# rafaelsoStanford/State_Policy_DiffusionModel

Measured on AMD Instinct MI355X. Metric: denoise-steps/sec (B=4096, horizon=32), higher is better.
Workload: dtype f32 (split-fp16 MFMA operands, fp32 accumulate)

## Files before the change

### state_policy_diffusionmodel_amd/csrc/conv_gemm.hip

```cpp
#include <algorithm>
#include <cstdlib>

#include "device_utils.h"

namespace spdm {

typedef float f32x16 __attribute__((ext_vector_type(16)));
typedef float f32x4 __attribute__((ext_vector_type(4)));
typedef float f32x2 __attribute__((ext_vector_type(2)));
typedef unsigned u32x2 __attribute__((ext_vector_type(2)));
typedef _Float16 f16x8 __attribute__((ext_vector_type(8)));
typedef _Float16 f16x4 __attribute__((ext_vector_type(4)));

constexpr float SPLIT_ACT_SCALE = 16.0f;
constexpr float SPLIT_DESCALE = 1.0f / 2048.0f;

typedef _Float16 f16x2 __attribute__((ext_vector_type(2)));
__device__ __forceinline__ f32x2 split_pair(float a, float b) {
    unsigned h, l;
    split_pair_f16(a * SPLIT_ACT_SCALE, b * SPLIT_ACT_SCALE, h, l);
    return f32x2{__builtin_bit_cast(float, h), __builtin_bit_cast(float, l)};
}

constexpr int CK = 32;
// ... 443 lines not shown
#undef SPDM_TRANSFORM_A_X
#undef SPDM_WRITE_A_X
#undef SPDM_DMA_W
#undef SPDM_WOFF
#undef SPDM_LOAD_A
#undef SPDM_LOAD_W
#undef SPDM_STORE_W
#undef SPDM_TRANSFORM_A
#undef SPDM_WRITE_A

    if (PREC == PREC_SPLIT) {
#pragma unroll
        for (int mt = 0; mt < MT; ++mt)
#pragma unroll
            for (int nt = 0; nt < NT; ++nt)
#pragma unroll
                for (int r = 0; r < 16; ++r) acc[mt][nt][r] *= SPLIT_DESCALE;
    }

    SPDM_STAMP()
    float* srow = smem;
    constexpr int SROW_FLOATS = M_T * WN * 2;
    float* otile = smem + SROW_FLOATS;
    const bool unit4 = !W2 && (HW & 3) == 0;
#pragma unroll
    for (int mt = 0; mt < MT; ++mt)
#pragma unroll
        for (int nt = 0; nt < NT; ++nt) {
            const int col_l = wn * NT * 32 + nt * 32 + li;
#pragma unroll
            for (int r = 0; r < 16; ++r) {
                const int row_l = SPDM_ROW(mt, (r & 3) + 8 * (r >> 2) + 4 * kh);
                otile[row_l * N_T + col_l] = acc[mt][nt][r];
            }
        }

    const int epi = (ksp > 1) ? EPI_PLAIN : a.epi;
    float* const dstp = (ksp > 1) ? a.partial + (size_t)ks * M * N : a.dst;
    const int dst_ld = (ksp > 1) ? N : a.dst_ld;
    if (epi == EPI_STATS) {
#pragma unroll
        for (int mt = 0; mt < MT; ++mt)
#pragma unroll
            for (int g = 0; g < 4; ++g) {
                const int r0 = wm * MT * 32 + mt * 32 + 8 * g + 4 * kh;
                if (unit4) {
                    float s1 = 0.f, s2 = 0.f;
#pragma unroll
                    for (int nt = 0; nt < NT; ++nt)
#pragma unroll
                        for (int j = 0; j < 4; ++j) {
                            const float v = acc[mt][nt][4 * g + j];
                            s1 += v;
                            s2 += v * v;
                        }
                    s1 = half_sum(s1);
                    s2 = half_sum(s2);
                    if (li == 0) {
                        srow[((r0 >> 2) * WN + wn) * 2] = s1;
                        srow[((r0 >> 2) * WN + wn) * 2 + 1] = s2;
                    }
                } else {
#pragma unroll
                    for (int j = 0; j < 4; ++j) {
                        float s1 = 0.f, s2 = 0.f;
#pragma unroll
                        for (int nt = 0; nt < NT; ++nt) {
                            const float v = acc[mt][nt][4 * g + j];
                            s1 += v;
                            s2 += v * v;
                        }
                        s1 = half_sum(s1);
                        s2 = half_sum(s2);
                        if (li == 0) {
                            const int rr = SPDM_ROW(mt, 8 * g + 4 * kh + j);
                            srow[(rr * WN + wn) * 2] = s1;
                            srow[(rr * WN + wn) * 2 + 1] = s2;
                        }
                    }
                }
            }
    }
    SPDM_STAMP()
    __syncthreads();
    SPDM_STAMP()

    if (epi == EPI_STATS) {
        const int t_lo = m0, t_hi = min(m0 + M_T, M);
        if (t_hi > t_lo) {
            const int b_first = t_lo / HW, b_last = (t_hi - 1) / HW;
            const int ush = unit4 ? 2 : 0;
            for (int t = tid; t <= b_last - b_first; t += NTHR) {
                const int b = b_first + t;
                const int r_lo = max(b * HW, t_lo) - m0, r_hi = min((b + 1) * HW, t_hi) - m0;
                double s1 = 0.0, s2 = 0.0;
                for (int u = r_lo >> ush; u < ((r_hi + (unit4 ? 3 : 0)) >> ush); ++u)
                    for (int w2 = 0; w2 < WN; ++w2) {
                        s1 += (double)srow[(u * WN + w2) * 2];
                        s2 += (double)srow[(u * WN + w2) * 2 + 1];
                    }
                const int slot = (mtile - (b * HW) / M_T) * n_ntiles + ntile;
                double* o = a.epi_stats + ((size_t)b * epi_slots + slot) * 2;
                o[0] = s1;
                o[1] = s2;
            }
        }
    }

    {
        constexpr int TPR = N_T / 4, RPP = NTHR / TPR;
        const int c4o = tid % TPR, r0 = tid / TPR;
        const bool has_bias = (epi == EPI_BIAS || epi == EPI_BIAS_GELU || epi == EPI_BIAS_RESID);
        f32x4 bias4 = {0.f, 0.f, 0.f, 0.f};
        if (has_bias) bias4 = *reinterpret_cast<const f32x4*>(a.bias + n0 + c4o * 4);
#pragma unroll 4
        for (int p = 0; p < M_T / RPP; ++p) {
            const int row_l = p * RPP + r0;
            const int row = m0 + row_l;
            if (row < M && !(dbg & DBG_NO_STORE)) {
                f32x4 v = *reinterpret_cast<const f32x4*>(otile + row_l * N_T + c4o * 4);
                v += bias4;
                if (epi == EPI_BIAS_GELU) {
                    v.x = gelu_erf(v.x); v.y = gelu_erf(v.y); v.z = gelu_erf(v.z); v.w = gelu_erf(v.w);
                }
                if (epi == EPI_BIAS_RESID)
                    v += *reinterpret_cast<const f32x4*>(a.resid + (size_t)row * a.resid_ld + n0 + c4o * 4);
                *reinterpret_cast<f32x4*>(dstp + (size_t)row * dst_ld + n0 + c4o * 4) = v;
                if (a.row_stats != nullptr) {
                    float s1 = (v.x + v.y) + (v.z + v.w);
                    float s2 = (v.x * v.x + v.y * v.y) + (v.z * v.z + v.w * v.w);
#pragma unroll
                    for (int o2 = TPR >> 1; o2 > 0; o2 >>= 1) {
                        s1 += __shfl_xor(s1, o2, 64);
                        s2 += __shfl_xor(s2, o2, 64);
                    }
                    if (c4o == 0) {
                        double* rs = a.row_stats + ((size_t)row * n_ntiles + ntile) * 2;
                        rs[0] = (double)s1;
                        rs[1] = (double)s2;
                    }
                }
            }
        }
    }
    SPDM_STAMP()
#ifdef SPDM_DIAG
    if (stamping) a.stamps[(tid >> 8) * 128 + 127] = (unsigned long long)nstamp;
#endif
#undef SPDM_STAMP
#undef SPDM_ROW
}

int spdm_tune(int idx, int dflt) {
    constexpr int NT = 24;
    static int val[NT];
    static bool have[NT], init = false;
    if (!init) {
        for (int i = 0; i < NT; ++i) {
            char name[20];
            snprintf(name, sizeof(name), "SPDM_TUNE%d", i);
            const char* e = getenv(name);
            have[i] = e != nullptr;
            val[i] = e ? atoi(e) : 0;
        }
        init = true;
    }
    return (idx >= 0 && idx < NT && have[idx]) ? val[idx] : dflt;
}

GemmGeom gemm_geometry(int M, int N, int K, int HW, int W, int taps, int split, unsigned sw, bool stats_epi) {
    GemmGeom g;
    g.skinny = 0;
    g.reg = 0;
    if (stats_epi && conv_reg_geometry(M, N, K, HW, W, taps, split, sw)) {
        g.reg = 1;
        g.m_tile = 64; g.n_tile = 64; g.n_tiles = 1; g.ksplit = 1;
        g.st_m_tile = 64; g.st_n_tiles = 1;
        g.slots = stats_slots(HW, 64, 1);
        return g;
    }
    if (stats_epi && taps != 1 && conv_skinny_geometry(M, N, K, HW, W, taps, split, sw, &g.m_tile, &g.n_tile)) {
        g.skinny = 1;
        g.ksplit = 1;
        g.n_tiles = N / g.n_tile;
        g.st_m_tile = g.m_tile;
        g.st_n_tiles = g.n_tiles;
        g.slots = stats_slots(HW, g.st_m_tile, g.st_n_tiles);
        return g;
    }
    if (stats_epi && split && taps != 1 && spdm_tune(5, 0) > 0) {
        g.m_tile = spdm_tune(5, 0);
        g.n_tile = spdm_tune(6, 64);
        g.ksplit = std::max(1, spdm_tune(7, 1));
        if (N % g.n_tile != 0 || (g.m_tile != 128 && g.m_tile != 256)) { g.n_tile = 64; g.m_tile = 128; }
        g.n_tiles = N / g.n_tile;
        if (g.ksplit > K / CK) g.ksplit = K / CK;
        while (g.ksplit > 1 && (size_t)g.ksplit * M * N * sizeof(float) > SPLITK_WORKSPACE_BYTES) --g.ksplit;
        if (g.ksplit > 1) { g.st_m_tile = combine_rows(HW, N); g.st_n_tiles = 1; }
        else { g.st_m_tile = g.m_tile; g.st_n_tiles = g.n_tiles; }
        g.slots = stats_slots(HW, g.st_m_tile, g.st_n_tiles);
        return g;
    }
    const int nt128 = (N % 128 == 0) ? N / 128 : 0;
    const int nt_pref = nt128 ? nt128 : N / 64;
    bool big = split && taps != 1 && M >= 256;
    if (big && (long long)((M + 255) / 256) * nt_pref < spdm_tune(4, nt128 ? 257 : 192)) big = false;
    if (big && taps == 3 && HW % 4 == 0 && (long long)((M + 255) / 256) * nt_pref < 512 && !(sw & SW_T3_BIG)) big = false;
    g.m_tile = big ? 256 : 128;
    g.n_tile = nt128 ? 128 : 64;
    if (!big && nt128 && (long long)((M + 127) / 128) * nt128 < 192) g.n_tile = 64;
    if (big && g.n_tile == 64 && taps == 9 && (long long)((M + 511) / 512) * (N / 64) >= 192 &&
        !(sw & SW_NO_T512) && ((HW & 3) != 0 || (sw & SW_T512)))
        g.m_tile = 512;
    g.n_tiles = N / g.n_tile;
    g.ksplit = 1;
    const bool may_split = stats_epi && split && taps != 1 && K % CK == 0 && !(sw & SW_NO_SPLITK);
    if (may_split && !big && split && taps == 9 && W == 2 && (HW & 7) == 0 && M >= 256 && K % 64 == 0 && K >= 256 && spdm_tune(2, 1) != 0) {
        const long long t256 = (long long)((M + 255) / 256) * nt_pref;
        const int target = spdm_tune(0, 256);
        int S = (int)std::min<long long>(K / 64, (target + t256 - 1) / t256);
        while (S > 1 && (size_t)S * M * N * sizeof(float) > SPLITK_WORKSPACE_BYTES) --S;
        if (t256 * S >= target * 3 / 4 && S <= spdm_tune(3, 8)) {
            g.m_tile = 256; g.n_tile = nt128 ? 128 : 64; g.n_tiles = N / g.n_tile; g.ksplit = S;
            if (S > 1) { g.st_m_tile = combine_rows(HW, N); g.st_n_tiles = 1; }
            else { g.st_m_tile = g.m_tile; g.st_n_tiles = g.n_tiles; }
            g.slots = stats_slots(HW, g.st_m_tile, g.st_n_tiles);
            return g;
        }
    }
    if (may_split && !big) {
        const int nchunks = K / CK;
        const int target = spdm_tune(0, 256);
        const bool wide128 = nt128 && (HW & 3) == 0 && K % 64 == 0 && !(sw & (SW_NO_WIDE | SW_NO_WIDE128)) && spdm_tune(1, 0) != 0;
        const long long mt = (M + 127) / 128;
        if (wide128 && mt * nt128 < target) g.n_tile = 128, g.n_tiles = nt128;
        const long long tiles = mt * g.n_tiles;
        if (tiles < target) {
            const bool pairs = g.n_tile == 128 && (HW & 3) == 0 && K % 64 == 0 && !(sw & (SW_NO_WIDE | SW_NO_WIDE128));
            const int unit = pairs ? 2 : 1;
            int S = (int)std::min<long long>(nchunks / unit, (target + tiles - 1) / tiles);
            while (S > 1 && (size_t)S * M * N * sizeof(float) > SPLITK_WORKSPACE_BYTES) --S;
            if (S > 1) g.ksplit = S;
        }
    }
    if (g.ksplit > 1) {
        g.st_m_tile = combine_rows(HW, N);
        g.st_n_tiles = 1;
    } else {
        g.st_m_tile = g.m_tile;
        g.st_n_tiles = g.n_tiles;
    }
    g.slots = stats_slots(HW, g.st_m_tile, g.st_n_tiles);
    return g;
}

GemmGeom gemm_geometry(const GemmArgs& a) {
    return gemm_geometry(a.geom_M > 0 ? a.geom_M : a.M, a.N, a.K, a.HW, a.W, a.taps, a.split, a.sw, a.epi == EPI_STATS && a.partial != nullptr);
}

bool gemm_takes_fused_source(const GemmArgs& a) {
    if (!(a.pro == PRO_POOL || a.pro == PRO_UPCAT) || !a.split || a.wgt_frag == nullptr || (a.sw & SW_NO_FUSED_SRC) || a.epi != EPI_STATS) return false;
    if (a.pro == PRO_UPCAT && (a.up_C <= 0 || a.up_C >= a.K || a.up_C % CK != 0 || (a.H & 1) || (a.W & 1))) return false;
    const GemmGeom g = gemm_geometry(a);
    if (g.skinny != 0) return true;
    if (a.pro != PRO_UPCAT || g.reg || g.ksplit > 1) return false;
    GemmArgs b = a;
    b.ksplit = 1;
    return conv_wide_takes_upcat(b, g);
}

bool gemm_takes_two_sources(const GemmArgs& a0) {
    if (a0.skip == nullptr || !a0.split || a0.wgt_frag == nullptr || (a0.sw & SW_NO_FUSED_SRC) || a0.epi != EPI_STATS) return false;
    GemmArgs a = a0;
    const GemmGeom g = gemm_geometry(a);
    if (g.skinny || g.reg || g.m_tile == 512) return false;
    a.ksplit = g.ksplit;
    return conv_wide_supported(a, g);
}

static bool uses_w2(const GemmArgs& a, const GemmGeom& g) {
    return a.split && g.m_tile == 256 && a.taps == 9 && a.W == 2 && a.HW % 2 == 0 && !(a.sw & SW_NO_W2);
}
static bool uses_wp4(const GemmArgs& a0, const GemmGeom& g) {
    if (!(a0.split && a0.taps == 9 && a0.W == 4 && g.n_tile == 128 && (g.m_tile == 128 || g.m_tile == 256) && a0.HW % 16 == 0 &&
          a0.K % 64 == 0 && !(a0.sw & SW_NO_WP4)) || g.skinny) return false;
    GemmArgs a = a0;
    a.ksplit = g.ksplit;
    return conv_wide_supported(a, g);
}
static bool uses_wp8(const GemmArgs& a0, const GemmGeom& g) {
    if (!(a0.split && a0.taps == 9 && a0.W == 8 && g.n_tile == 128 && g.m_tile == 256 && a0.HW % 32 == 0 && a0.K % 64 == 0 &&
          !(a0.sw & SW_NO_WP8)) || g.skinny) return false;
    GemmArgs a = a0;
    a.ksplit = g.ksplit;
    return conv_wide_supported(a, g);
}
double gemm_flops(const GemmArgs& a0) {
    GemmArgs a = a0;
    const GemmGeom g = gemm_geometry(a.geom_M > 0 ? a.geom_M : a.M, a.N, a.K, a.HW, a.W, a.taps, a.split, a.sw, a.epi == EPI_STATS);
    if (a.pro == PRO_UPCAT && !g.skinny && gemm_takes_fused_source(a0)) a.pro = a.skip_stats.p != nullptr ? PRO_GN : PRO_NONE;
    const double taps = uses_w2(a, g) ? 6.0 : uses_wp4(a, g) ? 7.5 : uses_wp8(a, g) ? 8.25 : (double)a.taps;
    return 2.0 * (double)a.M * (double)a.N * (double)a.K * taps;
}

template <bool HALO, int PREC, int WM, int WN, int MT, int NT, int TPI, bool W2 = false, bool DEEP = false>
static hipError_t launch_cfg(const GemmArgs& a, const GemmGeom& g, hipStream_t s) {
    constexpr int M_T = WM * MT * 32, N_T = WN * NT * 32, NTHR = WM * WN * 64;
// ... 107 lines not shown
```

### state_policy_diffusionmodel_amd/csrc/sa_tail.hip

```cpp
#include <algorithm>
#include <cstdlib>

#include "device_utils.h"

namespace spdm {

namespace {

typedef float tf32x4 __attribute__((ext_vector_type(4)));
typedef float tf32x2 __attribute__((ext_vector_type(2)));
typedef _Float16 tf16x8 __attribute__((ext_vector_type(8)));
typedef _Float16 tf16x2 __attribute__((ext_vector_type(2)));

constexpr float T_ACT_SCALE = 16.0f;
constexpr float T_DESCALE = 1.0f / 2048.0f;
constexpr int T_LDK = 36;
template <int C> struct TailShape {
    static_assert(C == 128 || C == 256, "C = 128 or 256");
    static constexpr int TM = 8192 / C;
    static constexpr int WM = TM / 32, WN = 4 / WM;
    static constexpr int NCH = C / 32;
    static constexpr int TPR = C / 4, RPP = 256 / TPR;
    static constexpr int NP = TM / RPP;
};
// ... 276 lines not shown
            const int prow = item / TPR, cq = item % TPR;
            const int r0 = (prow / Wo) * 2 * W + 2 * (prow % Wo);
            if (m0 + r0 < M) {
                const float* p = otile + r0 * T_C + cq * 4;
                const tf32x4 v00 = *reinterpret_cast<const tf32x4*>(p), v01 = *reinterpret_cast<const tf32x4*>(p + T_C);
                const tf32x4 v10 = *reinterpret_cast<const tf32x4*>(p + W * T_C), v11 = *reinterpret_cast<const tf32x4*>(p + (W + 1) * T_C);
                tf32x4 m;
#pragma unroll
                for (int e = 0; e < 4; ++e) m[e] = fmaxf(fmaxf(v00[e], v01[e]), fmaxf(v10[e], v11[e]));
                *reinterpret_cast<tf32x4*>(a.pool + (size_t)(m0 / 4 + prow) * T_C + cq * 4) = m;
            }
        }
    }
    TAIL_STAMP(8)
}

struct SaQkvArgs {
    const float* x; float* qkv; int M;
    const float* wf;
    const float *b_in, *ln_g, *ln_b;
    const float* ab; int L;
    FilmSpec fs;
};

template <int C>
__global__ __launch_bounds__(256, 2) void sa_qkv_kernel(const SaQkvArgs a) {
    using S = TailShape<C>;
    constexpr int T_C = C, T_M = S::TM, NCH = S::NCH, RPP = S::RPP, TPR = S::TPR;
    constexpr int RT = 2, CT = 4;
    constexpr int NP = S::NP;
    extern __shared__ __attribute__((aligned(16))) float smem[];
    const int tid = threadIdx.x, lane = tid & 63;
    const int wave = __builtin_amdgcn_readfirstlane(tid >> 6);
    const int wm = wave / S::WN, wn = wave % S::WN, l16 = lane & 15, kg = lane >> 4;
    const int M = a.M;
    const int m0 = blockIdx.x * T_M;
    float* Abuf = smem;
    float* otile = smem;
    const int c16 = tid % TPR, srow0 = tid / TPR;
    const int aoff0 = (wm * 32 + l16) * T_LDK + kg * 4;
    const size_t wlane = ((size_t)(wn * CT) * 2) * 256 + lane * 4;
    constexpr size_t WCHUNK = (size_t)(3 * C / 16) * 2 * 256;
    constexpr size_t WPROD = (size_t)(C / 16) * 2 * 256;
    tf16x8 fb[2][CT][2], fa[2][2];
    tf32x4 acc[RT][CT], v[NP];

    const int g_lo = (int)blockIdx.y * 3 / (int)gridDim.y, g_hi = ((int)blockIdx.y + 1) * 3 / (int)gridDim.y;
    TAIL_LOAD_B(0, a.wf + (size_t)g_lo * WPROD, 0)
    {
        const tf32x4 g4 = *reinterpret_cast<const tf32x4*>(a.ln_g + c16 * 4);
        const tf32x4 b4 = *reinterpret_cast<const tf32x4*>(a.ln_b + c16 * 4);
#pragma unroll
        for (int i = 0; i < NP; ++i) {
            const int row = min(m0 + RPP * i + srow0, M - 1);
            v[i] = *reinterpret_cast<const tf32x4*>(a.x + (size_t)row * T_C + c16 * 4);
        }
        if (a.ab != nullptr) tail_film_fold<C>(v, a.ab, a.L, m0, M, c16, srow0);
        if (a.fs.on) {
            float* abl = smem + NCH * T_M * T_LDK;
            tail_film_rows<C>(a.fs, a.L, m0, M, wave, lane, abl);
            __syncthreads();
            tail_film_fold_lds<C>(v, abl, a.L, m0, M, c16, srow0);
        }
        float part[NP];
#pragma unroll
        for (int i = 0; i < NP; ++i) part[i] = (v[i].x + v[i].y) + (v[i].z + v[i].w);
#pragma unroll
        for (int i = 0; i < NP; ++i) part[i] = row16_sum_dpp(part[i]);
#pragma unroll
        for (int i = 0; i < NP; ++i) part[i] = sum_xor16(part[i]);
        if (TPR == 64) {
#pragma unroll
            for (int i = 0; i < NP; ++i) part[i] = sum_xor32(part[i]);
        }
#pragma unroll
        for (int i = 0; i < NP; ++i) {
            const float mean = part[i] * (1.0f / (float)C);
            const tf32x4 t = v[i];
            const tf32x4 d = {t.x - mean, t.y - mean, t.z - mean, t.w - mean};
            v[i] = d;
            part[i] = (d.x * d.x + d.y * d.y) + (d.z * d.z + d.w * d.w);
        }
#pragma unroll
        for (int i = 0; i < NP; ++i) part[i] = row16_sum_dpp(part[i]);
#pragma unroll
        for (int i = 0; i < NP; ++i) part[i] = sum_xor16(part[i]);
        if (TPR == 64) {
#pragma unroll
            for (int i = 0; i < NP; ++i) part[i] = sum_xor32(part[i]);
        }
#pragma unroll
        for (int i = 0; i < NP; ++i) {
            const float rstd = __builtin_amdgcn_rsqf(part[i] * (1.0f / (float)C) + 1e-5f);
            const tf32x4 d = v[i];
            v[i] = tf32x4{d.x * rstd * g4.x + b4.x, d.y * rstd * g4.y + b4.y, d.z * rstd * g4.z + b4.z, d.w * rstd * g4.w + b4.w};
        }
    }
    TAIL_WRITE_SLAB(v)
    __syncthreads();
    for (int g = g_lo; g < g_hi; ++g) {
        const float* wg = a.wf + (size_t)g * WPROD;
        const float* wnext = a.wf + (size_t)(g < 2 ? g + 1 : g) * WPROD;
        const tf32x4 bi = *reinterpret_cast<const tf32x4*>(a.b_in + g * T_C + c16 * 4);
        TAIL_GEMM(wg, wnext)
        {
            float* ot = smem + NCH * T_M * T_LDK;
            if (g > g_lo) __syncthreads();
#pragma unroll
            for (int rt_ = 0; rt_ < RT; ++rt_)
#pragma unroll
                for (int ct_ = 0; ct_ < CT; ++ct_) {
                    const int col_ = wn * 64 + ct_ * 16 + l16;
#pragma unroll
                    for (int j_ = 0; j_ < 4; ++j_)
                        ot[(wm * 32 + rt_ * 16 + 4 * kg + j_) * T_C + col_] = acc[rt_][ct_][j_] * T_DESCALE;
                }
            __syncthreads();
#pragma unroll
            for (int i = 0; i < NP; ++i) {
                const int r = RPP * i + srow0;
                if (m0 + r < M) {
                    tf32x4 t = *reinterpret_cast<const tf32x4*>(ot + r * T_C + c16 * 4);
                    t += bi;
                    *reinterpret_cast<tf32x4*>(a.qkv + (size_t)(m0 + r) * (3 * T_C) + g * T_C + c16 * 4) = t;
                }
            }
        }
    }
    (void)otile;
}

struct SaHeadArgs {
    const float* x; float* att; int M;
    const float* wf;
    const float *b_in, *ln_g, *ln_b;
    const float* ab; int L;
    FilmSpec fs;
};

__device__ __forceinline__ float row16_max_dpp(float v) {
#define DPP_MAX(ctrl_) v = fmaxf(v, __builtin_bit_cast(float, __builtin_amdgcn_update_dpp(0, __builtin_bit_cast(int, v), ctrl_, 0xf, 0xf, false)));
    DPP_MAX(0xB1) DPP_MAX(0x4E) DPP_MAX(0x141) DPP_MAX(0x140)
#undef DPP_MAX
    return v;
}
__device__ __forceinline__ float head_exp_neg(float x) {
    const float t = x * 1.44269504f;
    const float tl = __fmaf_rn(x, 1.44269504f, -t) + x * 1.925963033e-8f;
    return __builtin_amdgcn_exp2f(t) * (1.0f + tl * 0.69314718f);
}

#undef TAIL_SPLIT2
#define TAIL_SPLIT2 tsplit2_plain
template <int C>
__global__ __launch_bounds__(256, 2) void sa_head_kernel(const SaHeadArgs a) {
    using S = TailShape<C>;
    constexpr int T_C = C, T_M = S::TM, NCH = S::NCH, RPP = S::RPP, TPR = S::TPR;
    constexpr int NP = S::NP;
    constexpr int D = C / 4;
    constexpr int QROW = 2 * D + 8;
    constexpr int VROW = 2 * T_M + 8;
    constexpr int NKT = T_M / 16;
    constexpr int NDT = D / 16;
    static_assert(T_M * VROW <= 2 * T_M * QROW, "P aliases the q / k tiles");
    extern __shared__ __attribute__((aligned(16))) float smem[];
    const int tid = threadIdx.x, lane = tid & 63;
    const int wave = __builtin_amdgcn_readfirstlane(tid >> 6);
    const int l16 = lane & 15, kg = lane >> 4;
    const int M = a.M, L = a.L;
    const int m0 = blockIdx.x * T_M;
    float* Abuf = smem;
    _Float16* Qs = reinterpret_cast<_Float16*>(smem + NCH * T_M * T_LDK);
    _Float16* Ks = Qs + T_M * QROW;
    _Float16* Vt = Ks + T_M * QROW;
    _Float16* Ps = Qs;
    const int c16 = tid % TPR, srow0 = tid / TPR;

    {
        tf32x4 v[NP];
        const tf32x4 g4 = *reinterpret_cast<const tf32x4*>(a.ln_g + c16 * 4);
        const tf32x4 b4 = *reinterpret_cast<const tf32x4*>(a.ln_b + c16 * 4);
#pragma unroll
        for (int i = 0; i < NP; ++i) {
            const int row = min(m0 + RPP * i + srow0, M - 1);
            v[i] = *reinterpret_cast<const tf32x4*>(a.x + (size_t)row * T_C + c16 * 4);
        }
        if (a.ab != nullptr) tail_film_fold<C>(v, a.ab, a.L, m0, M, c16, srow0);
        if (a.fs.on) {
            float* abl = reinterpret_cast<float*>(Qs);
            tail_film_rows<C>(a.fs, a.L, m0, M, wave, lane, abl);
            __syncthreads();
            tail_film_fold_lds<C>(v, abl, a.L, m0, M, c16, srow0);
            __syncthreads();
        }
        float part[NP];
#pragma unroll
        for (int i = 0; i < NP; ++i) part[i] = (v[i].x + v[i].y) + (v[i].z + v[i].w);
#pragma unroll
        for (int i = 0; i < NP; ++i) part[i] = trow_sum<TPR>(part[i]);
#pragma unroll
        for (int i = 0; i < NP; ++i) {
            const float mean = part[i] * (1.0f / (float)C);
            const tf32x4 t = v[i];
            const tf32x4 d = {t.x - mean, t.y - mean, t.z - mean, t.w - mean};
            v[i] = d;
            part[i] = (d.x * d.x + d.y * d.y) + (d.z * d.z + d.w * d.w);
        }
#pragma unroll
        for (int i = 0; i < NP; ++i) part[i] = trow_sum<TPR>(part[i]);
#pragma unroll
        for (int i = 0; i < NP; ++i) {
            const float rstd = __builtin_amdgcn_rsqf(part[i] * (1.0f / (float)C) + 1e-5f);
            const tf32x4 d = v[i];
            v[i] = tf32x4{d.x * rstd * g4.x + b4.x, d.y * rstd * g4.y + b4.y, d.z * rstd * g4.z + b4.z, d.w * rstd * g4.w + b4.w};
        }
        TAIL_WRITE_SLAB(v)
    }
    __syncthreads();

    const int rtw = (C == 128) ? wave : (wave >> 1);
    const int cpw = (C == 128) ? 0 : (wave & 1);
    const bool attn_wave = wave < NKT;
    const float qscale = (D == 32) ? 0.17677669529663687f : 0.125f;
    constexpr size_t WCHUNK = (size_t)(3 * C / 16) * 2 * 256;

    tf16x8 fbw[2][2][2];
#define HEAD_WPTR(h_, g_) (a.wf + ((size_t)((g_) * (C / 16) + (h_) * (D / 16) + cpw * 2) * 2) * 256 + lane * 4)
#define HEAD_LOAD_W(slot_, wp_, kc_)                                                                 \
    _Pragma("unroll") for (int ct_ = 0; ct_ < 2; ++ct_) {                                           \
        fbw[slot_][ct_][0] = *reinterpret_cast<const tf16x8*>((wp_) + (size_t)(kc_) * WCHUNK + ct_ * 512);        \
        fbw[slot_][ct_][1] = *reinterpret_cast<const tf16x8*>((wp_) + (size_t)(kc_) * WCHUNK + ct_ * 512 + 256);  \
    }
    HEAD_LOAD_W(0, HEAD_WPTR(0, 0), 0)
    for (int h = 0; h < 4; ++h) {
#pragma unroll
        for (int g = 0; g < 3; ++g) {
            tf32x4 acc[2] = {tf32x4{0.f, 0.f, 0.f, 0.f}, tf32x4{0.f, 0.f, 0.f, 0.f}};
            const float* wp = HEAD_WPTR(h, g);
            const float* wnext = (g < 2) ? HEAD_WPTR(h, g + 1) : HEAD_WPTR(min(h + 1, 3), 0);
#pragma unroll
            for (int kc = 0; kc < NCH; ++kc) {
                if (kc + 1 < NCH) { HEAD_LOAD_W((kc + 1) & 1, wp, kc + 1) } else { HEAD_LOAD_W(0, wnext, 0) }
                const float* ap = Abuf + (kc * T_M + rtw * 16 + l16) * T_LDK + kg * 4;
                const tf16x8 a_h = *reinterpret_cast<const tf16x8*>(ap), a_l = *reinterpret_cast<const tf16x8*>(ap + 16);
#pragma unroll
                for (int ct = 0; ct < 2; ++ct) {
                    acc[ct] = __builtin_amdgcn_mfma_f32_16x16x32_f16(a_h, fbw[kc & 1][ct][0], acc[ct], 0, 0, 0);
                    acc[ct] = __builtin_amdgcn_mfma_f32_16x16x32_f16(a_h, fbw[kc & 1][ct][1], acc[ct], 0, 0, 0);
                    acc[ct] = __builtin_amdgcn_mfma_f32_16x16x32_f16(a_l, fbw[kc & 1][ct][0], acc[ct], 0, 0, 0);
                }
            }
#pragma unroll
            for (int ct = 0; ct < 2; ++ct) {
                const int col = cpw * 32 + ct * 16 + l16;
                const float bias = a.b_in[g * T_C + h * D + col];
#pragma unroll
                for (int j = 0; j < 4; ++j) {
                    const int row = rtw * 16 + 4 * kg + j;
                    float val = acc[ct][j] * T_DESCALE + bias;
                    if (g == 0) val *= qscale;
                    const float xs = val * T_ACT_SCALE;
                    const _Float16 hi = (_Float16)xs, lo = (_Float16)(xs - (float)hi);
                    if (g == 2) { Vt[col * VROW + row] = hi; Vt[col * VROW + T_M + row] = lo; }
                    else { _Float16* X = (g == 0) ? Qs : Ks; X[row * QROW + col] = hi; X[row * QROW + D + col] = lo; }
                }
            }
        }
        __syncthreads();

        tf32x4 sc[NKT];
#pragma unroll
        for (int kt = 0; kt < NKT; ++kt) sc[kt] = tf32x4{0.f, 0.f, 0.f, 0.f};
        if (attn_wave) {
#pragma unroll
            for (int ks = 0; ks < D / 32; ++ks) {
                const _Float16* qp = Qs + (wave * 16 + l16) * QROW + 32 * ks + 8 * kg;
                const tf16x8 q_h = *reinterpret_cast<const tf16x8*>(qp), q_l = *reinterpret_cast<const tf16x8*>(qp + D);
#pragma unroll
                for (int kt = 0; kt < NKT; ++kt) {
                    const _Float16* kp = Ks + (kt * 16 + l16) * QROW + 32 * ks + 8 * kg;
                    const tf16x8 k_h = *reinterpret_cast<const tf16x8*>(kp), k_l = *reinterpret_cast<const tf16x8*>(kp + D);
                    sc[kt] = __builtin_amdgcn_mfma_f32_16x16x32_f16(q_h, k_h, sc[kt], 0, 0, 0);
                    sc[kt] = __builtin_amdgcn_mfma_f32_16x16x32_f16(q_h, k_l, sc[kt], 0, 0, 0);
                    sc[kt] = __builtin_amdgcn_mfma_f32_16x16x32_f16(q_l, k_h, sc[kt], 0, 0, 0);
                }
            }
        }
        __syncthreads();

        if (attn_wave) {
#pragma unroll
            for (int j = 0; j < 4; ++j) {
                const int row = wave * 16 + 4 * kg + j;
                const int smp = row / L;
                float s[NKT];
                float mx = -3.0e38f;
#pragma unroll
                for (int kt = 0; kt < NKT; ++kt) {
                    const bool own = ((kt * 16 + l16) / L) == smp;
                    s[kt] = own ? sc[kt][j] * (1.0f / 256.0f) : -3.0e38f;
                    mx = fmaxf(mx, s[kt]);
                }
                mx = row16_max_dpp(mx);
                float sum = 0.f;
#pragma unroll
                for (int kt = 0; kt < NKT; ++kt) {
                    s[kt] = (s[kt] > -1.0e38f) ? head_exp_neg(s[kt] - mx) : 0.f;
                    sum += s[kt];
                }
                sum = row16_sum_dpp(sum);
                const float inv = 1024.0f / sum;
#pragma unroll
                for (int kt = 0; kt < NKT; ++kt) {
                    const float ps = s[kt] * inv;
                    const _Float16 hi = (_Float16)ps, lo = (_Float16)(ps - (float)hi);
                    Ps[row * VROW + kt * 16 + l16] = hi;
                    Ps[row * VROW + T_M + kt * 16 + l16] = lo;
                }
            }
        }
        __syncthreads();

        if (attn_wave) {
            tf32x4 o[NDT];
#pragma unroll
            for (int dt = 0; dt < NDT; ++dt) o[dt] = tf32x4{0.f, 0.f, 0.f, 0.f};
#pragma unroll
            for (int ks = 0; ks < T_M / 32; ++ks) {
                const _Float16* pp = Ps + (wave * 16 + l16) * VROW + 32 * ks + 8 * kg;
                const tf16x8 p_h = *reinterpret_cast<const tf16x8*>(pp), p_l = *reinterpret_cast<const tf16x8*>(pp + T_M);
#pragma unroll
                for (int dt = 0; dt < NDT; ++dt) {
                    const _Float16* vp = Vt + (dt * 16 + l16) * VROW + 32 * ks + 8 * kg;
                    const tf16x8 v_h = *reinterpret_cast<const tf16x8*>(vp), v_l = *reinterpret_cast<const tf16x8*>(vp + T_M);
                    o[dt] = __builtin_amdgcn_mfma_f32_16x16x32_f16(p_h, v_h, o[dt], 0, 0, 0);
                    o[dt] = __builtin_amdgcn_mfma_f32_16x16x32_f16(p_h, v_l, o[dt], 0, 0, 0);
                    o[dt] = __builtin_amdgcn_mfma_f32_16x16x32_f16(p_l, v_h, o[dt], 0, 0, 0);
                }
            }
#pragma unroll
            for (int dt = 0; dt < NDT; ++dt)
#pragma unroll
                for (int j = 0; j < 4; ++j) {
                    const int row = m0 + wave * 16 + 4 * kg + j;
                    if (row < M) a.att[(size_t)row * T_C + h * D + dt * 16 + l16] = o[dt][j] * (1.0f / 16384.0f);
                }
        }
        __syncthreads();
    }
#undef TAIL_LOAD_B
#undef TAIL_LOAD_FA
#undef TAIL_WRITE_SLAB
#undef TAIL_GEMM
#undef TAIL_ACC_TO_TILE
}

}

#ifdef SPDM_DIAG_TAIL
extern "C" int spdm_debug_tail_stamps(unsigned long long* out64) {
    return hipMemcpyFromSymbol(out64, HIP_SYMBOL(g_tail_stamps), sizeof(unsigned long long) * 64) == hipSuccess ? 0 : -1;
}
#endif

bool sa_tail_supported(int C, unsigned sw) { return (C == 128 || C == 256) && !(sw & SW_NO_SA_TAIL); }

static int film_rows_cap(int TM, int L) { return (TM + L - 2) / L + 1; }
bool sa_tail_film_local(int C, int L) {
    if (!(C == 128 || C == 256) || L < 1) return false;
    return (size_t)film_rows_cap(8192 / C, L) * 2 * C * sizeof(float) <= (size_t)24 * 1024;
}

bool sa_tail_pools(int C, int L, int W, int rows) {
    if (!(C == 128 || C == 256) || W < 2 || (W & 1) || L <= 0 || rows <= 0) return false;
    return L % (2 * W) == 0 && (8192 / C) % (2 * W) == 0 && rows % L == 0;
}

hipError_t launch_sa_tail(int C, const float* o, const float* x, float* out, int rows, const float* wf_o, const float* wf_1,
                          const float* wf_2, const float* b_o, const float* b_1, const float* b_2, const float* ln_g,
                          const float* ln_b, const float* ab, int L, hipStream_t s, const FilmSpec* fs, SaRoute* route, float* pool,
                          int W) {
    if (fs && (ab || L <= 0 || !sa_tail_film_local(C, L) || fs->C != C)) return hipErrorInvalidValue;
    if (rows <= 0 || (ab && L <= 0) || !o || !x || !out || !wf_o || !wf_1 || !wf_2 || !b_o || !b_1 || !b_2 || !ln_g || !ln_b)
        return hipErrorInvalidValue;
    if (C != 128 && C != 256) return hipErrorInvalidValue;
    if (pool && !sa_tail_pools(C, L, W, rows)) return hipErrorInvalidValue;
    SaTailArgs a{};
    a.o = o; a.x = x; a.out = out; a.M = rows;
    a.wf_o = wf_o; a.wf_1 = wf_1; a.wf_2 = wf_2;
    a.b_o = b_o; a.b_1 = b_1; a.b_2 = b_2; a.ln_g = ln_g; a.ln_b = ln_b; a.ab = ab; a.L = L;
    a.pool = pool; a.W = W;
    if (fs) { a.fs = *fs; a.fs.on = 1; }
    const int TM = 8192 / C;
    const size_t lds = (size_t)(C / 32) * TM * T_LDK * sizeof(float)
                       + (fs ? (size_t)film_rows_cap(TM, L) * 2 * C * sizeof(float) : 0);
    if (route) { route->kernel = SA_ROUTE_TAIL; route->waves = 4; route->grid = (rows + TM - 1) / TM; if (route->dry) return hipSuccess; }
    if (C == 128) hipLaunchKernelGGL(sa_tail_kernel<128>, dim3((rows + TM - 1) / TM), dim3(256), lds, s, a);
    else hipLaunchKernelGGL(sa_tail_kernel<256>, dim3((rows + TM - 1) / TM), dim3(256), lds, s, a);
    return hipGetLastError();
}

bool sa_head_supported(int C, int L, unsigned sw) {
    return (C == 128 || C == 256) && L >= 1 && (8192 / C) % L == 0 && !(sw & (SW_NO_SA_TAIL | SW_NO_SA_HEAD));
}

hipError_t launch_sa_head(int C, const float* x, float* att, int rows, const float* wf_in, const float* b_in, const float* ln_g,
                          const float* ln_b, const float* ab, int L, hipStream_t s, const FilmSpec* fs, SaRoute* route) {
    if (rows <= 0 || !x || !att || !wf_in || !b_in || !ln_g || !ln_b || !sa_head_supported(C, L, 0) || rows % L != 0) return hipErrorInvalidValue;
    if (fs && (ab || !sa_tail_film_local(C, L) || fs->C != C)) return hipErrorInvalidValue;
    SaHeadArgs a{};
    a.x = x; a.att = att; a.M = rows; a.wf = wf_in; a.b_in = b_in; a.ln_g = ln_g; a.ln_b = ln_b; a.ab = ab; a.L = L;
    if (fs) { a.fs = *fs; a.fs.on = 1; }
    const int TM = 8192 / C, D = C / 4;
    const size_t lds = (size_t)(C / 32) * TM * T_LDK * sizeof(float) + ((size_t)2 * TM * (2 * D + 8) + (size_t)D * (2 * TM + 8)) * sizeof(_Float16);
    if (fs && (size_t)film_rows_cap(TM, L) * 2 * C * sizeof(float) > ((size_t)2 * TM * (2 * D + 8) + (size_t)D * (2 * TM + 8)) * sizeof(_Float16)) return hipErrorInvalidValue;
    const void* kern = C == 128 ? reinterpret_cast<const void*>(sa_head_kernel<128>) : reinterpret_cast<const void*>(sa_head_kernel<256>);
    const int tiles = (rows + TM - 1) / TM;
    if (route) { route->kernel = SA_ROUTE_HEAD; route->waves = 4; route->grid = tiles; if (route->dry) return hipSuccess; }
    if (hipError_t e = allow_full_lds(kern); e != hipSuccess) return e;
    if (C == 128) hipLaunchKernelGGL(sa_head_kernel<128>, dim3(tiles), dim3(256), lds, s, a);
    else hipLaunchKernelGGL(sa_head_kernel<256>, dim3(tiles), dim3(256), lds, s, a);
    return hipGetLastError();
}

hipError_t launch_sa_qkv(int C, const float* x, float* qkv, int rows, const float* wf_in, const float* b_in, const float* ln_g,
                         const float* ln_b, const float* ab, int L, hipStream_t s, const FilmSpec* fs, SaRoute* route) {
    if (fs && (ab || L <= 0 || !sa_tail_film_local(C, L) || fs->C != C)) return hipErrorInvalidValue;
    if (rows <= 0 || (ab && L <= 0) || !x || !qkv || !wf_in || !b_in || !ln_g || !ln_b) return hipErrorInvalidValue;
    if (C != 128 && C != 256) return hipErrorInvalidValue;
    SaQkvArgs a{};
    a.x = x; a.qkv = qkv; a.M = rows; a.wf = wf_in; a.b_in = b_in; a.ln_g = ln_g; a.ln_b = ln_b; a.ab = ab; a.L = L;
    if (fs) { a.fs = *fs; a.fs.on = 1; }
    const int TM = 8192 / C;
    const size_t lds = (size_t)((C / 32) * TM * T_LDK + TM * C) * sizeof(float);
    const void* kern = C == 128 ? reinterpret_cast<const void*>(sa_qkv_kernel<128>) : reinterpret_cast<const void*>(sa_qkv_kernel<256>);
    const int tiles = (rows + TM - 1) / TM;
    const int gy = (tiles < spdm_tune(15, 512)) ? 3 : 1;
    if (route) { route->kernel = SA_ROUTE_QKV; route->waves = 4; route->grid = tiles * gy; if (route->dry) return hipSuccess; }
    if (hipError_t e = allow_full_lds(kern); e != hipSuccess) return e;
    if (C == 128) hipLaunchKernelGGL(sa_qkv_kernel<128>, dim3(tiles, gy), dim3(256), lds, s, a);
    else hipLaunchKernelGGL(sa_qkv_kernel<256>, dim3(tiles, gy), dim3(256), lds, s, a);
    return hipGetLastError();
}

}
```

Before: 543,300.

## Run self-attention head per wave with register-resident Q/K/V operands

Adds a per-wave variant of the SA head kernel in which each of the 4 waves owns one attention head. It computes that head's Q, K and V projections directly into MFMA operand registers, then does the masked softmax and the PV product without staging Q/K/V/P through LDS or block-wide syncs. The LDS request shrinks to the slab plus an optional FiLM region, which may raise occupancy. The cost is heavy register pressure from the large operand arrays, which risks spills. The serial path stays available behind a tune switch, and the per-wave path is the default for both C values.

```diff
diff --git a/state_policy_diffusionmodel_amd/csrc/conv_gemm.hip b/state_policy_diffusionmodel_amd/csrc/conv_gemm.hip
--- a/state_policy_diffusionmodel_amd/csrc/conv_gemm.hip
+++ b/state_policy_diffusionmodel_amd/csrc/conv_gemm.hip
@@ -619,7 +619,7 @@
 }
 
 int spdm_tune(int idx, int dflt) {
-    constexpr int NT = 24;
+    constexpr int NT = 25;
     static int val[NT];
     static bool have[NT], init = false;
     if (!init) {
diff --git a/state_policy_diffusionmodel_amd/csrc/sa_tail.hip b/state_policy_diffusionmodel_amd/csrc/sa_tail.hip
--- a/state_policy_diffusionmodel_amd/csrc/sa_tail.hip
+++ b/state_policy_diffusionmodel_amd/csrc/sa_tail.hip
@@ -452,8 +452,22 @@
 
 #undef TAIL_SPLIT2
 #define TAIL_SPLIT2 tsplit2_plain
-template <int C>
-__global__ __launch_bounds__(256, 2) void sa_head_kernel(const SaHeadArgs a) {
+__device__ __forceinline__ float max_xor16(float v) {
+    const unsigned u = __builtin_bit_cast(unsigned, v);
+    const auto r = __builtin_amdgcn_permlane16_swap(u, u, false, false);
+    return fmaxf(__builtin_bit_cast(float, (unsigned)r[0]), __builtin_bit_cast(float, (unsigned)r[1]));
+}
+typedef unsigned tu32x4 __attribute__((ext_vector_type(4)));
+__device__ __forceinline__ void head_split8(const float (&x)[8], tf16x8& hi, tf16x8& lo) {
+    tu32x4 h, l;
+#pragma unroll
+    for (int i = 0; i < 4; ++i) { unsigned hh, ll; split_pair_f16(x[2 * i], x[2 * i + 1], hh, ll); h[i] = hh; l[i] = ll; }
+    hi = __builtin_bit_cast(tf16x8, h);
+    lo = __builtin_bit_cast(tf16x8, l);
+}
+
+template <int C, bool WAVES>
+__device__ __forceinline__ void sa_head_body(const SaHeadArgs& a) {
     using S = TailShape<C>;
     constexpr int T_C = C, T_M = S::TM, NCH = S::NCH, RPP = S::RPP, TPR = S::TPR;
     constexpr int NP = S::NP;
@@ -518,6 +532,157 @@
     }
     __syncthreads();
 
+    if constexpr (WAVES) {
+        constexpr int NDS = D / 32;
+        constexpr int NKS = T_M / 32;
+        constexpr int NCT = 2;
+        constexpr int NPS = NDT / NCT;
+        constexpr int RING = 3;
+        const int h = wave;
+        const float qscale = (D == 32) ? 0.17677669529663687f : 0.125f;
+        constexpr size_t WCHUNK = (size_t)(3 * C / 16) * 2 * 256;
+        tf16x8 Kop[NKT][NDS][2], Qop[NKT][NDS][2], Vop[NDT][NKS][2];
+        tf16x8 fbw[RING][NCT][2];
+#define HEADW_LOAD_W(t_)                                                                             \
+    {                                                                                                \
+        const float* wp_ = a.wf + ((size_t)(((t_) / (NPS * NCH)) * (C / 16) + h * (D / 16) + (((t_) / NCH) % NPS) * NCT) * 2) * 256 \
+                           + (size_t)((t_) % NCH) * WCHUNK + lane * 4;                               \
+        _Pragma("unroll") for (int ct_ = 0; ct_ < NCT; ++ct_) {                                     \
+            fbw[(t_) % RING][ct_][0] = *reinterpret_cast<const tf16x8*>(wp_ + ct_ * 512);            \
+            fbw[(t_) % RING][ct_][1] = *reinterpret_cast<const tf16x8*>(wp_ + ct_ * 512 + 256);      \
+        }                                                                                            \
+    }
+#pragma unroll
+        for (int t0 = 0; t0 < RING - 1; ++t0) HEADW_LOAD_W(t0)
+#pragma unroll
+        for (int g = 0; g < 3; ++g) {
+#pragma unroll
+            for (int p = 0; p < NPS; ++p) {
+                const float* bp = a.b_in + g * T_C + h * D + 16 * NCT * p;
+                tf32x4 acc[NCT][NKT];
+#pragma unroll
+                for (int ct = 0; ct < NCT; ++ct)
+#pragma unroll
+                    for (int tt = 0; tt < NKT; ++tt) acc[ct][tt] = tf32x4{0.f, 0.f, 0.f, 0.f};
+#pragma unroll
+                for (int kc = 0; kc < NCH; ++kc) {
+                    const int t = (g * NPS + p) * NCH + kc;
+                    if (t + RING - 1 < 3 * NPS * NCH) HEADW_LOAD_W(t + RING - 1)
+#pragma unroll
+                    for (int tt = 0; tt < NKT; ++tt) {
+                        const float* ap = Abuf + (kc * T_M + tt * 16 + l16) * T_LDK + kg * 4;
+                        const tf16x8 x_h = *reinterpret_cast<const tf16x8*>(ap), x_l = *reinterpret_cast<const tf16x8*>(ap + 16);
+#pragma unroll
+                        for (int ct = 0; ct < NCT; ++ct) {
+                            const tf16x8 w_h = fbw[t % RING][ct][0], w_l = fbw[t % RING][ct][1];
+                            if (g < 2) {
+                                acc[ct][tt] = __builtin_amdgcn_mfma_f32_16x16x32_f16(w_h, x_h, acc[ct][tt], 0, 0, 0);
+                                acc[ct][tt] = __builtin_amdgcn_mfma_f32_16x16x32_f16(w_l, x_h, acc[ct][tt], 0, 0, 0);
+                                acc[ct][tt] = __builtin_amdgcn_mfma_f32_16x16x32_f16(w_h, x_l, acc[ct][tt], 0, 0, 0);
+                            } else {
+                                acc[ct][tt] = __builtin_amdgcn_mfma_f32_16x16x32_f16(x_h, w_h, acc[ct][tt], 0, 0, 0);
+                                acc[ct][tt] = __builtin_amdgcn_mfma_f32_16x16x32_f16(x_h, w_l, acc[ct][tt], 0, 0, 0);
+                                acc[ct][tt] = __builtin_amdgcn_mfma_f32_16x16x32_f16(x_l, w_h, acc[ct][tt], 0, 0, 0);
+                            }
+                        }
+                    }
+                    __builtin_amdgcn_sched_barrier(0);
+                }
+                if (g < 2) {
+#pragma unroll
+                    for (int s2 = 0; s2 < NCT / 2; ++s2) {
+                        tf32x4 bias[2] = {*reinterpret_cast<const tf32x4*>(bp + 32 * s2 + 4 * kg), *reinterpret_cast<const tf32x4*>(bp + 32 * s2 + 16 + 4 * kg)};
+                        if (g == 1) { bias[0] *= T_ACT_SCALE; bias[1] *= T_ACT_SCALE; }
+#pragma unroll
+                        for (int tt = 0; tt < NKT; ++tt) {
+                            float xs[8];
+#pragma unroll
+                            for (int c2 = 0; c2 < 2; ++c2)
+#pragma unroll
+                                for (int j = 0; j < 4; ++j)
+                                    xs[4 * c2 + j] = (g == 0) ? __fmaf_rn(acc[2 * s2 + c2][tt][j], T_DESCALE, bias[c2][j]) * (qscale * T_ACT_SCALE)
+                                                              : __fmaf_rn(acc[2 * s2 + c2][tt][j], T_DESCALE * T_ACT_SCALE, bias[c2][j]);
+                            if (g == 0) head_split8(xs, Qop[tt][p * (NCT / 2) + s2][0], Qop[tt][p * (NCT / 2) + s2][1]);
+                            else head_split8(xs, Kop[tt][p * (NCT / 2) + s2][0], Kop[tt][p * (NCT / 2) + s2][1]);
+                        }
+                    }
+                } else {
+#pragma unroll
+                    for (int ct = 0; ct < NCT; ++ct) {
+                        const float bias = bp[16 * ct + l16] * T_ACT_SCALE;
+#pragma unroll
+                        for (int ks = 0; ks < NKS; ++ks) {
+                            float xs[8];
+#pragma unroll
+                            for (int t2 = 0; t2 < 2; ++t2)
+#pragma unroll
+                                for (int j = 0; j < 4; ++j) xs[4 * t2 + j] = __fmaf_rn(acc[ct][2 * ks + t2][j], T_DESCALE * T_ACT_SCALE, bias);
+                            head_split8(xs, Vop[NCT * p + ct][ks][0], Vop[NCT * p + ct][ks][1]);
+                        }
+                    }
+                }
+            }
+        }
+#undef HEADW_LOAD_W
+#pragma unroll
+        for (int qt = 0; qt < NKT; ++qt) {
+            tf32x4 sc[NKT];
+#pragma unroll
+            for (int kt = 0; kt < NKT; ++kt) {
+                sc[kt] = tf32x4{0.f, 0.f, 0.f, 0.f};
+#pragma unroll
+                for (int s = 0; s < NDS; ++s) {
+                    sc[kt] = __builtin_amdgcn_mfma_f32_16x16x32_f16(Kop[kt][s][0], Qop[qt][s][0], sc[kt], 0, 0, 0);
+                    sc[kt] = __builtin_amdgcn_mfma_f32_16x16x32_f16(Kop[kt][s][1], Qop[qt][s][0], sc[kt], 0, 0, 0);
+                    sc[kt] = __builtin_amdgcn_mfma_f32_16x16x32_f16(Kop[kt][s][0], Qop[qt][s][1], sc[kt], 0, 0, 0);
+                }
+            }
+            const unsigned qx = (unsigned)((4 * kg) ^ (qt * 16 + l16));
+            float mx = -3.0e38f;
+#pragma unroll
+            for (int kt = 0; kt < NKT; ++kt)
+#pragma unroll
+                for (int j = 0; j < 4; ++j) {
+                    const bool own = ((unsigned)(kt * 16 + j) ^ qx) < (unsigned)L;
+                    sc[kt][j] = own ? sc[kt][j] * (1.0f / 256.0f) : -3.0e38f;
+                    mx = fmaxf(mx, sc[kt][j]);
+                }
+            mx = max_xor32(max_xor16(mx));
+            float sum = 0.f;
+#pragma unroll
+            for (int kt = 0; kt < NKT; ++kt)
+#pragma unroll
+                for (int j = 0; j < 4; ++j) {
+                    sc[kt][j] = (sc[kt][j] > -1.0e38f) ? head_exp_neg(sc[kt][j] - mx) : 0.f;
+                    sum += sc[kt][j];
+                }
+            sum = sum_xor32(sum_xor16(sum));
+            const float inv = 1024.0f / sum;
+            tf16x8 Pop[NKS][2];
+#pragma unroll
+            for (int ks = 0; ks < NKS; ++ks) {
+                float ps[8];
+#pragma unroll
+                for (int t2 = 0; t2 < 2; ++t2)
+#pragma unroll
+                    for (int j = 0; j < 4; ++j) ps[4 * t2 + j] = sc[2 * ks + t2][j] * inv;
+                head_split8(ps, Pop[ks][0], Pop[ks][1]);
+            }
+            const int row = m0 + qt * 16 + l16;
+#pragma unroll
+            for (int dt = 0; dt < NDT; ++dt) {
+                tf32x4 o = {0.f, 0.f, 0.f, 0.f};
+#pragma unroll
+                for (int ks = 0; ks < NKS; ++ks) {
+                    o = __builtin_amdgcn_mfma_f32_16x16x32_f16(Vop[dt][ks][0], Pop[ks][0], o, 0, 0, 0);
+                    o = __builtin_amdgcn_mfma_f32_16x16x32_f16(Vop[dt][ks][1], Pop[ks][0], o, 0, 0, 0);
+                    o = __builtin_amdgcn_mfma_f32_16x16x32_f16(Vop[dt][ks][0], Pop[ks][1], o, 0, 0, 0);
+                }
+                if (row < M) *reinterpret_cast<tf32x4*>(a.att + (size_t)row * T_C + h * D + dt * 16 + 4 * kg) = o * (1.0f / 16384.0f);
+            }
+        }
+        (void)Vt; (void)Ps; (void)Ks;
+    } else {
     const int rtw = (C == 128) ? wave : (wave >> 1);
     const int cpw = (C == 128) ? 0 : (wave & 1);
     const bool attn_wave = wave < NKT;
@@ -648,12 +813,18 @@
         }
         __syncthreads();
     }
+    }
 #undef TAIL_LOAD_B
 #undef TAIL_LOAD_FA
 #undef TAIL_WRITE_SLAB
 #undef TAIL_GEMM
 #undef TAIL_ACC_TO_TILE
 }
+
+template <int C>
+__global__ __launch_bounds__(256, 2) void sa_head_kernel(const SaHeadArgs a) { sa_head_body<C, true>(a); }
+template <int C>
+__global__ __launch_bounds__(256, 2) void sa_head_serial_kernel(const SaHeadArgs a) { sa_head_body<C, false>(a); }
 
 }
 
@@ -712,14 +883,24 @@
     a.x = x; a.att = att; a.M = rows; a.wf = wf_in; a.b_in = b_in; a.ln_g = ln_g; a.ln_b = ln_b; a.ab = ab; a.L = L;
     if (fs) { a.fs = *fs; a.fs.on = 1; }
     const int TM = 8192 / C, D = C / 4;
-    const size_t lds = (size_t)(C / 32) * TM * T_LDK * sizeof(float) + ((size_t)2 * TM * (2 * D + 8) + (size_t)D * (2 * TM + 8)) * sizeof(_Float16);
-    if (fs && (size_t)film_rows_cap(TM, L) * 2 * C * sizeof(float) > ((size_t)2 * TM * (2 * D + 8) + (size_t)D * (2 * TM + 8)) * sizeof(_Float16)) return hipErrorInvalidValue;
-    const void* kern = C == 128 ? reinterpret_cast<const void*>(sa_head_kernel<128>) : reinterpret_cast<const void*>(sa_head_kernel<256>);
+    const bool per_wave = (spdm_tune(24, 3) >> (C == 256 ? 1 : 0)) & 1;
+    const size_t slab = (size_t)(C / 32) * TM * T_LDK * sizeof(float);
+    const size_t film = (size_t)film_rows_cap(TM, L) * 2 * C * sizeof(float);
+    const size_t qkv = ((size_t)2 * TM * (2 * D + 8) + (size_t)D * (2 * TM + 8)) * sizeof(_Float16);
+    const size_t lds = slab + (per_wave ? (fs ? film : 0) : qkv);
+    if (fs && !per_wave && film > qkv) return hipErrorInvalidValue;
+    const void* kern = per_wave ? (C == 128 ? reinterpret_cast<const void*>(sa_head_kernel<128>) : reinterpret_cast<const void*>(sa_head_kernel<256>))
+                                : (C == 128 ? reinterpret_cast<const void*>(sa_head_serial_kernel<128>) : reinterpret_cast<const void*>(sa_head_serial_kernel<256>));
     const int tiles = (rows + TM - 1) / TM;
     if (route) { route->kernel = SA_ROUTE_HEAD; route->waves = 4; route->grid = tiles; if (route->dry) return hipSuccess; }
     if (hipError_t e = allow_full_lds(kern); e != hipSuccess) return e;
-    if (C == 128) hipLaunchKernelGGL(sa_head_kernel<128>, dim3(tiles), dim3(256), lds, s, a);
-    else hipLaunchKernelGGL(sa_head_kernel<256>, dim3(tiles), dim3(256), lds, s, a);
+    if (per_wave) {
+        if (C == 128) hipLaunchKernelGGL(sa_head_kernel<128>, dim3(tiles), dim3(256), lds, s, a);
+        else hipLaunchKernelGGL(sa_head_kernel<256>, dim3(tiles), dim3(256), lds, s, a);
+    } else {
+        if (C == 128) hipLaunchKernelGGL(sa_head_serial_kernel<128>, dim3(tiles), dim3(256), lds, s, a);
+        else hipLaunchKernelGGL(sa_head_serial_kernel<256>, dim3(tiles), dim3(256), lds, s, a);
+    }
     return hipGetLastError();
 }
 
```

New measurement: 555,300, median of 6. +2.2%, better.
